# ruiminshen/yolo2-pytorch

Measured on AMD Instinct MI355X. Metric: images/sec (416x416) train+detect, Darknet-19 YOLOv2: value = TRAIN step, batch 64 per GPU (configs[2]) at every N; detect (configs[1]) = roofline.detect_images_per_sec, higher is better.
Workload: dtype f32; 1 GPU; Darknet-19 YOLOv2 20-class train 416x416 batch-64/GPU: fwd + region loss + bwd + SGD (BASELINE configs[2]); classes=20, global_batch=64, parallelism=single GPU, weights=random-init seed 0 (bench_data.randomize)

## Files before the change

include/yolo2_hip.h:

```cpp
#ifndef YOLO2_HIP_H
#define YOLO2_HIP_H

#include <stdint.h>

#ifdef __cplusplus
extern "C" {
#endif

#define Y2_OK 0
#define Y2_EINVAL (-1)
#define Y2_EALIGN (-2)
#define Y2_ENOSUP (-3)

#define Y2_STATS_REPL 32

typedef void* y2_stream_t;

int y2_abi_version(void);
const char* y2_build_info(void);


int y2_pack_weight(const float* w, float* dst, int Cout, int Cin, int ksize, int mode, y2_stream_t stream);

#define Y2_PREP_FPROP 0
// ... 161 lines not shown

int y2_bn_act_fwd(const float* z, const float* scale, const float* shift, float slope, float* y, float* y_pool,
                  int B, int H, int W, int C, int ldz, int ldy, int coff, int ldp, int poff, int out_mode, y2_stream_t stream);

int y2_bn_act_bwd(const float* z, const float* scale, const float* shift, const float* mean, const float* invstd, const float* gamma,
                  float slope, const float* dy_full, int ldf, int foff, int fmode, const float* dy_pool, int ldp, int poff,
                  double* sums, float* dz, int ldd, int B, int H, int W, int C, int ldz, int has_bn, y2_stream_t stream);

int y2_bn_act_fwd_ex(const float* z, const float* scale, const float* shift, float slope, const float* residual, int ldr, float* y, float* y_pool,
                     int B, int H, int W, int C, int ldz, int ldy, int coff, int ldp, int poff, int out_mode, y2_stream_t stream);
int y2_bn_act_bwd_ex(const float* z, const float* scale, const float* shift, const float* mean, const float* invstd, const float* gamma,
                     float slope, const float* dy_full, int ldf, int foff, int fmode, const float* dy_pool, int ldp, int poff,
                     const float* dy_full2, int ld2, const float* residual, int ldr, float* dres, int lddr,
                     double* sums, float* dz, int ldd, int B, int H, int W, int C, int ldz, int has_bn, y2_stream_t stream);

long long y2_wino6_tiles(int32_t B, int32_t H, int32_t W);
int y2_bn_act_bwd_wino6(const float* z, const float* scale, const float* shift, const float* mean, const float* invstd, const float* gamma,
                        float slope, const float* dy_full, int ldf, int foff, double* sums, float* v6, float* m6, float* dz, int ldd,
                        int B, int H, int W, int C, int ldz, int has_bn, y2_stream_t stream);

int y2_maxpool_bwd(const float* x, const float* dy, const float* dy2, float* dx, int B, int H, int W, int C, int ldx, int ldy, int lddx,
                   int ksize, int stride, int pad, int pad_end, y2_stream_t stream);

int y2_colsum(const float* x, long long M, int C, int ld, double* out, y2_stream_t stream);
int y2_f64_to_f32(const double* src, float* dst, int n, double mul, y2_stream_t stream);

int y2_decode_bwd(const float* iou, const float* center_offset, const float* d_iou, const float* d_center_offset, const float* d_size_norm,
                  const float* d_logits, float* d_feature, int boxes, int C, y2_stream_t stream);

int y2_region_loss_fwd(const float* iou, const float* center_offset, const float* size_norm, const float* logits,
// ... 41 lines not shown
```

yolo2-pytorch_amd/_hip.py:

```python
import ctypes
import os
import subprocess

import torch

_HERE = os.path.dirname(os.path.abspath(__file__))
LIB_PATH = os.environ.get('Y2_LIB') or os.path.join(_HERE, 'csrc', 'libyolo2_hip.so')
_lib = None

c_int, c_float, c_void_p = ctypes.c_int, ctypes.c_float, ctypes.c_void_p


class ConvParams(ctypes.Structure):
    _fields_ = [('x', c_void_p), ('w', c_void_p), ('scale', c_void_p), ('shift', c_void_p),
                ('y', c_void_p), ('y_pool', c_void_p), ('stats', c_void_p),
                ('B', ctypes.c_int32), ('H', ctypes.c_int32), ('W', ctypes.c_int32),
                ('Cin', ctypes.c_int32), ('ldx', ctypes.c_int32), ('Cout', ctypes.c_int32), ('ksize', ctypes.c_int32),
                ('ldy', ctypes.c_int32), ('coff', ctypes.c_int32), ('ldp', ctypes.c_int32), ('poff', ctypes.c_int32),
                ('out_mode', ctypes.c_int32), ('slope', c_float), ('tile', ctypes.c_int32),
                ('workspace', c_void_p), ('workspace_bytes', ctypes.c_int64),
                ('residual', c_void_p), ('ldr', ctypes.c_int32), ('stride', ctypes.c_int32), ('pad_plus1', ctypes.c_int32),
                ('transposed', ctypes.c_int32), ('out_h', ctypes.c_int32), ('out_w', ctypes.c_int32), ('algo', ctypes.c_int32),
                ('w_plane', ctypes.c_int64)]

# ... 57 lines not shown
    'y2_filter_visible': [c_void_p, c_void_p, c_int, c_int, c_int, c_int, c_float, c_void_p, c_void_p, c_void_p, c_void_p, c_void_p],
    'y2_iou_matrix': [c_void_p, c_void_p, c_void_p, c_void_p, c_int, c_int, c_int, c_float, c_int, c_void_p, c_void_p],
    'y2_iou_pair': [c_void_p, c_void_p, c_void_p, c_void_p, c_int, c_float, c_void_p, c_void_p],
    'y2_conv_wgrad': [c_void_p, c_void_p, c_void_p, c_int, c_int, c_int, c_int, c_int, c_int, c_int, c_int, c_void_p],
    'y2_conv_wgrad_ex': [c_void_p, c_void_p, c_void_p, c_int, c_int, c_int, c_int, c_int, c_int, c_int, c_int, c_int, c_int, c_void_p],
    'y2_conv0_wgrad_fused': [c_void_p] * 7 + [c_float, c_void_p, c_int, c_void_p, c_void_p] + [c_int] * 7 + [c_void_p],
    'y2_conv0_wgrad': [c_void_p, c_void_p, c_void_p, c_int, c_int, c_int, c_int, c_int, c_int, c_void_p],
    'y2_bn_finalize': [c_void_p, ctypes.c_double, c_void_p, c_void_p, c_void_p, c_void_p, c_float, c_float, c_void_p, c_void_p, c_void_p, c_void_p, c_int, c_void_p, c_void_p],
    'y2_bn_act_fwd': [c_void_p, c_void_p, c_void_p, c_float, c_void_p, c_void_p, c_int, c_int, c_int, c_int, c_int, c_int, c_int, c_int, c_int, c_int, c_void_p],
    'y2_bn_act_bwd': [c_void_p, c_void_p, c_void_p, c_void_p, c_void_p, c_void_p, c_float, c_void_p, c_int, c_int, c_int, c_void_p, c_int, c_int,
                      c_void_p, c_void_p, c_int, c_int, c_int, c_int, c_int, c_int, c_int, c_void_p],
    'y2_bn_act_fwd_ex': [c_void_p, c_void_p, c_void_p, c_float, c_void_p, c_int, c_void_p, c_void_p, c_int, c_int, c_int, c_int, c_int, c_int, c_int, c_int, c_int, c_int, c_void_p],
    'y2_bn_act_bwd_ex': [c_void_p, c_void_p, c_void_p, c_void_p, c_void_p, c_void_p, c_float, c_void_p, c_int, c_int, c_int, c_void_p, c_int, c_int,
                         c_void_p, c_int, c_void_p, c_int, c_void_p, c_int,
                         c_void_p, c_void_p, c_int, c_int, c_int, c_int, c_int, c_int, c_int, c_void_p],
    'y2_wino6_tiles': [c_int, c_int, c_int],
    'y2_bn_act_bwd_wino6': [c_void_p, c_void_p, c_void_p, c_void_p, c_void_p, c_void_p, c_float, c_void_p, c_int, c_int, c_void_p, c_void_p, c_void_p, c_void_p, c_int,
                            c_int, c_int, c_int, c_int, c_int, c_int, c_void_p],
    'y2_maxpool_bwd': [c_void_p, c_void_p, c_void_p, c_void_p, c_int, c_int, c_int, c_int, c_int, c_int, c_int, c_int, c_int, c_int, c_int, c_void_p],
    'y2_colsum': [c_void_p, ctypes.c_longlong, c_int, c_int, c_void_p, c_void_p],
    'y2_dwconv_fwd': [c_void_p, c_void_p, c_void_p, c_void_p, c_float, c_void_p, c_void_p, c_int, c_int, c_int, c_int, c_int, c_int, c_int, c_void_p],
    'y2_dwconv_dgrad': [c_void_p, c_void_p, c_void_p, c_int, c_int, c_int, c_int, c_int, c_int, c_int, c_void_p],
    'y2_dwconv_wgrad': [c_void_p, c_void_p, c_void_p, c_void_p, ctypes.c_longlong, c_int, c_int, c_int, c_int, c_int, c_int, c_int, c_void_p],
    'y2_dwconv_wgrad_workspace_bytes': [c_int, c_int, c_int, c_int, c_int],
    'y2_f64_to_f32': [c_void_p, c_void_p, c_int, ctypes.c_double, c_void_p],
    'y2_decode_bwd': [c_void_p, c_void_p, c_void_p, c_void_p, c_void_p, c_void_p, c_void_p, c_int, c_int, c_void_p],
    'y2_region_loss_fwd': [c_void_p] * 11 + [c_int] * 6 + [c_float] + [c_void_p] * 5 + [c_void_p],
    'y2_region_loss_finalize': [c_void_p, ctypes.c_double, c_int, c_void_p, c_void_p],
    'y2_region_loss_bwd': [c_void_p] * 9 + [c_int] * 6 + [c_float] + [c_void_p] * 5 + [c_void_p] * 4 + [c_void_p],
    'y2_nms_host': [c_void_p, c_void_p, c_void_p, c_void_p, c_void_p, c_int, c_int, c_float, c_int, c_void_p, c_void_p],
# ... 653 lines not shown
```

yolo2-pytorch_amd/csrc/train.hip:

```cpp
#include "common.h"

namespace {

inline int stream_grid(long long total, int block, int cap_mult = 8) {
    long long g = (total + block - 1) / block;
    const long long cap = (long long)Y2_NUM_CU * cap_mult;
    return (int)(g < 1 ? 1 : (g > cap ? cap : g));
}

__global__ void bn_finalize_kernel(const double* __restrict__ stats, double n, const float* gamma, const float* beta,
                                   float* running_mean, float* running_var, float momentum, float eps,
                                   float* scale, float* shift, float* mean_out, float* invstd_out, int C, long long* num_batches_tracked) {
    const int c = blockIdx.x * blockDim.x + threadIdx.x;
    if (c >= C) return;
    if (c == 0 && num_batches_tracked != nullptr) *num_batches_tracked += 1;
    double s1 = 0.0, s2 = 0.0;
    for (int r = 0; r < Y2_STATS_REPL; ++r) { s1 += stats[(size_t)r * 2 * C + c]; s2 += stats[(size_t)r * 2 * C + C + c]; }
    const double mean = s1 / n;
    double var = s2 / n - mean * mean;
    if (var < 0.0) var = 0.0;
    const float invstd = (float)(1.0 / sqrt(var + (double)eps));
    const float s = gamma[c] * invstd;
    scale[c] = s;
    shift[c] = beta[c] - (float)mean * s;
    mean_out[c] = (float)mean;
    invstd_out[c] = invstd;
    if (running_mean != nullptr) {
        const double unbiased = n > 1.0 ? var * n / (n - 1.0) : var;
        running_mean[c] = (1.f - momentum) * running_mean[c] + momentum * (float)mean;
        running_var[c] = (1.f - momentum) * running_var[c] + momentum * (float)unbiased;
    }
}

struct ActArgs {
    const float* z; const float* scale; const float* shift;
    float* y; float* y_pool;
    int B, H, W, C, ldz, ldy, coff, ldp, poff, out_mode;
    float slope;
    const float* res; int ldr;
    y2_fastdiv d_wo, d_ho;
};

__device__ __forceinline__ float act1(float z, float sc, float sh, float slope) {
    const float u = z * sc + sh;
    return u > 0.f ? u : u * slope;
}

__device__ __forceinline__ void act_decode(uint32_t p, const y2_fastdiv& d_wo, const y2_fastdiv& d_ho, int Wo, int Ho, int& b, int& yo, int& xo) {
    const uint32_t r = y2_div(p, d_wo);
    xo = (int)(p - r * (uint32_t)Wo);
    const uint32_t bb = y2_div(r, d_ho);
    yo = (int)(r - bb * (uint32_t)Ho);
    b = (int)bb;
}
// ... 1 lines not shown
template <bool POOL, int CV>
__global__ void bn_act_fwd_kernel(const ActArgs a, long long total) {
    const int Cg = a.C / CV;
    const int Wo = POOL ? a.W / 2 : a.W, Ho = POOL ? a.H / 2 : a.H;
    const long long tid = (long long)blockIdx.x * blockDim.x + threadIdx.x;
    const long long nthreads = (long long)gridDim.x * blockDim.x;
    const int c = (int)(tid % Cg) * CV;
    const uint32_t npix = (uint32_t)(total / Cg), pstep = (uint32_t)(nthreads / Cg);
    float sc[CV], sh[CV];
#pragma unroll
    for (int e = 0; e < CV; ++e) { sc[e] = a.scale ? a.scale[c + e] : 1.f; sh[e] = a.shift ? a.shift[c + e] : 0.f; }
    const bool need_yx = POOL || a.out_mode == 1;
    for (uint32_t p = (uint32_t)(tid / Cg); p < npix; p += pstep) {
        int b = 0, yo = 0, xo = 0;
        if (need_yx) act_decode(p, a.d_wo, a.d_ho, Wo, Ho, b, yo, xo);
        float pm[CV];
#pragma unroll
        for (int q = 0; q < (POOL ? 4 : 1); ++q) {
            const int yy = POOL ? 2 * yo + (q >> 1) : yo, xx = POOL ? 2 * xo + (q & 1) : xo;
            const long long pix = need_yx ? ((long long)b * a.H + yy) * a.W + xx : (long long)p;
            float v[CV];
            if (CV == 4) {
                const f32x4 zz = *reinterpret_cast<const f32x4*>(a.z + pix * a.ldz + c);
                f32x4 rr = {0.f, 0.f, 0.f, 0.f};
                if (a.res != nullptr) rr = *reinterpret_cast<const f32x4*>(a.res + pix * a.ldr + c);
#pragma unroll
                for (int e = 0; e < 4; ++e) { const float u = zz[e] * sc[e] + sh[e] + rr[e]; v[e] = u > 0.f ? u : u * a.slope; }
            } else {
                const float u = a.z[pix * a.ldz + c] * sc[0] + sh[0] + (a.res != nullptr ? a.res[pix * a.ldr + c] : 0.f);
                v[0] = u > 0.f ? u : u * a.slope;
            }
            if (a.y != nullptr) {
                long long o;
                if (a.out_mode == 1) {
                    o = (((long long)b * (a.H >> 1) + (yy >> 1)) * (a.W >> 1) + (xx >> 1)) * a.ldy + a.coff + ((yy & 1) * 2 + (xx & 1)) * a.C + c;
                } else {
                    o = pix * a.ldy + a.coff + c;
                }
                if (CV == 4) { f32x4 w = {v[0], v[1], v[2], v[3]}; *reinterpret_cast<f32x4*>(a.y + o) = w; }
                else a.y[o] = v[0];
            }
#pragma unroll
            for (int e = 0; e < CV; ++e) pm[e] = (q == 0) ? v[e] : fmaxf(pm[e], v[e]);
        }
        if (POOL && a.y_pool != nullptr) {
            const long long o = (long long)p * a.ldp + a.poff + c;
            if (CV == 4) { f32x4 w = {pm[0], pm[1], pm[2], pm[3]}; *reinterpret_cast<f32x4*>(a.y_pool + o) = w; }
            else a.y_pool[o] = pm[0];
        }
    }
}

struct ActBwdArgs {
    const float* z; const float* scale; const float* shift; const float* mean; const float* invstd; const float* gamma;
    const float* dy_full; const float* dy_pool;
    const float* dy_full2; int ld2;
    const float* res; int ldr;
    float* dres; int lddr;
    double* sums;
    float* partial;
    float* block_partial;
    float* dz;
    int B, H, W, C, ldz, ldf, foff, fmode, ldp, poff, ldd;
    float slope;
    double n;
    int has_bn;
    y2_fastdiv d_wo, d_ho;
};

template <bool POOL, int CV, bool APPLY>
// ... 14 lines not shown
        sc[e] = a.scale ? a.scale[c + e] : 1.f; sh[e] = a.shift ? a.shift[c + e] : 0.f;
        mu[e] = a.has_bn ? a.mean[c + e] : 0.f; is[e] = a.has_bn ? a.invstd[c + e] : 1.f;
        if (APPLY && a.has_bn == 1) {
            gs[e] = a.gamma[c + e] * is[e];
            ma[e] = (float)(a.sums[c + e] / a.n);
            mb[e] = (float)(a.sums[a.C + c + e] / a.n);
        } else if (APPLY && a.has_bn == 2) {
            gs[e] = a.gamma[c + e] * is[e]; ma[e] = 0.f; mb[e] = 0.f;
        } else { gs[e] = 1.f; ma[e] = 0.f; mb[e] = 0.f; }
    }
    float s1[CV], s2[CV];
#pragma unroll
    for (int e = 0; e < CV; ++e) { s1[e] = 0.f; s2[e] = 0.f; }

    const uint32_t npix = (uint32_t)(total / Cg), pstep = (uint32_t)(nthreads / Cg);
    const bool need_yx = POOL || a.fmode == 1;
    for (uint32_t p = (uint32_t)(tid / Cg); p < npix; p += pstep) {
        int b = 0, yo = 0, xo = 0;
        if (need_yx) act_decode(p, a.d_wo, a.d_ho, Wo, Ho, b, yo, xo);
        float zv[POOL ? 4 : 1][CV], yv[POOL ? 4 : 1][CV];
        long long pixs[POOL ? 4 : 1];
#pragma unroll
        for (int q = 0; q < (POOL ? 4 : 1); ++q) {
            const int yy = POOL ? 2 * yo + (q >> 1) : yo, xx = POOL ? 2 * xo + (q & 1) : xo;
            pixs[q] = need_yx ? ((long long)b * a.H + yy) * a.W + xx : (long long)p;
            if (CV == 4) {
                const f32x4 zz = *reinterpret_cast<const f32x4*>(a.z + pixs[q] * a.ldz + c);
#pragma unroll
                for (int e = 0; e < 4; ++e) zv[q][e] = zz[e];
            } else zv[q][0] = a.z[pixs[q] * a.ldz + c];
#pragma unroll
            for (int e = 0; e < CV; ++e) yv[q][e] = zv[q][e] * sc[e] + sh[e];
// ... 653 lines not shown
    return (int)(((want + unit - 1) / unit) * unit);
}

}

extern "C" int y2_bn_finalize(const double* stats, double count, const float* gamma, const float* beta,
                              float* running_mean, float* running_var, float momentum, float eps,
                              float* scale, float* shift, float* mean, float* invstd, int C, long long* num_batches_tracked, y2_stream_t stream) {
    if (!stats || !gamma || !beta || !scale || !shift || !mean || !invstd || C <= 0 || count <= 0) return Y2_EINVAL;
    Y2_LAUNCH("bn_finalize_kernel", 0.0, bn_finalize_kernel, dim3(y2_cdiv(C, 256)), dim3(256), 0, y2_s(stream), stats, count, gamma, beta, running_mean, running_var,
                       momentum, eps, scale, shift, mean, invstd, C, num_batches_tracked);
    Y2_LAUNCH_CHECK();
    return Y2_OK;
}

extern "C" int y2_bn_act_fwd_ex(const float* z, const float* scale, const float* shift, float slope, const float* residual, int ldr, float* y, float* y_pool,
                                int B, int H, int W, int C, int ldz, int ldy, int coff, int ldp, int poff, int out_mode, y2_stream_t stream) {
    if (!z || (!y && !y_pool) || B <= 0 || H <= 0 || W <= 0 || C <= 0) return Y2_EINVAL;
    const bool pool = y_pool != nullptr;
    if ((pool || out_mode == 1) && ((H & 1) || (W & 1))) return Y2_EINVAL;
    ActArgs a;
    a.z = z; a.scale = scale; a.shift = shift; a.y = y; a.y_pool = y_pool;
    a.B = B; a.H = H; a.W = W; a.C = C; a.ldz = ldz; a.ldy = ldy; a.coff = coff; a.ldp = ldp; a.poff = poff; a.out_mode = out_mode; a.slope = slope;
    a.res = residual; a.ldr = ldr;
    if (residual != nullptr && ldr < C) return Y2_EINVAL;
    const bool vec = (!residual || (!(ldr & 3) && y2_aligned16(residual))) && !(C & 3) && !(ldz & 3) && (!y || (!(ldy & 3) && !(coff & 3) && y2_aligned16(y))) && (!pool || (!(ldp & 3) && !(poff & 3) && y2_aligned16(y_pool))) && y2_aligned16(z);
    const long long pix = (long long)B * (pool ? H / 2 : H) * (pool ? W / 2 : W);
    if (pix >= 0x7fffffffLL || C > 8192) return Y2_ENOSUP;
    const long long total = pix * (vec ? C / 4 : C);
    const int grid = act_grid(total, vec ? C / 4 : C);
    a.d_wo = y2_make_fastdiv((uint32_t)(pool ? W / 2 : W)); a.d_ho = y2_make_fastdiv((uint32_t)(pool ? H / 2 : H));
    hipStream_t s = y2_s(stream);
    if (pool) { if (vec) Y2_LAUNCH("bn_act_fwd_kernel", 0.0, (bn_act_fwd_kernel<true, 4>), dim3(grid), dim3(256), 0, s, a, total); else Y2_LAUNCH("bn_act_fwd_kernel", 0.0, (bn_act_fwd_kernel<true, 1>), dim3(grid), dim3(256), 0, s, a, total); }
    else { if (vec) Y2_LAUNCH("bn_act_fwd_kernel", 0.0, (bn_act_fwd_kernel<false, 4>), dim3(grid), dim3(256), 0, s, a, total); else Y2_LAUNCH("bn_act_fwd_kernel", 0.0, (bn_act_fwd_kernel<false, 1>), dim3(grid), dim3(256), 0, s, a, total); }
    Y2_LAUNCH_CHECK();
    return Y2_OK;
}

static int bn_act_bwd_impl(const float* z, const float* scale, const float* shift, const float* mean, const float* invstd, const float* gamma,
                           float slope, const float* dy_full, int ldf, int foff, int fmode, const float* dy_pool, int ldp, int poff,
                           const float* dy_full2, int ld2, const float* residual, int ldr, float* dres, int lddr,
                           double* sums, float* dz, int ldd, int B, int H, int W, int C, int ldz, int has_bn, y2_stream_t stream, float* park, long long park_floats) {
    if (!z || (!dy_full && !dy_pool) || !sums || B <= 0 || H <= 0 || W <= 0 || C <= 0) return Y2_EINVAL;
    if (dz == nullptr && dres != nullptr) return Y2_EINVAL;
    if (has_bn < 0 || has_bn > 2 || (has_bn && (!mean || !invstd || !gamma))) return Y2_EINVAL;
    const bool pool = dy_pool != nullptr;
    if ((pool || fmode == 1) && ((H & 1) || (W & 1))) return Y2_EINVAL;
    if (C > 8192) return Y2_ENOSUP;
    ActBwdArgs a;
    a.z = z; a.scale = scale; a.shift = shift; a.mean = mean; a.invstd = invstd; a.gamma = gamma;
    a.dy_full = dy_full; a.dy_pool = dy_pool; a.sums = sums; a.dz = dz;
    a.B = B; a.H = H; a.W = W; a.C = C; a.ldz = ldz; a.ldf = ldf; a.foff = foff; a.fmode = fmode; a.ldp = ldp; a.poff = poff; a.ldd = ldd;
    a.slope = slope; a.n = (double)B * H * W; a.has_bn = has_bn;
    a.dy_full2 = dy_full2; a.ld2 = ld2; a.res = residual; a.ldr = ldr; a.dres = dres; a.lddr = lddr;
    const bool vec = (!dy_full2 || (!(ld2 & 3) && y2_aligned16(dy_full2))) && (!residual || (!(ldr & 3) && y2_aligned16(residual))) && (!dres || (!(lddr & 3) && y2_aligned16(dres))) && !(C & 3) && !(ldz & 3) && (!dz || (!(ldd & 3) && y2_aligned16(dz))) && y2_aligned16(z) &&
                     (!dy_full || (!(ldf & 3) && !(foff & 3) && y2_aligned16(dy_full))) && (!pool || (!(ldp & 3) && !(poff & 3) && y2_aligned16(dy_pool)));
    const int Cg = vec ? C / 4 : C;
    const long long pix = (long long)B * (pool ? H / 2 : H) * (pool ? W / 2 : W);
    if (pix >= 0x7fffffffLL) return Y2_ENOSUP;
    const long long total = pix * Cg;
    const int grid = act_grid(total, Cg);
    a.d_wo = y2_make_fastdiv((uint32_t)(pool ? W / 2 : W)); a.d_ho = y2_make_fastdiv((uint32_t)(pool ? H / 2 : H));
    const size_t lds = (size_t)2 * C * sizeof(float);
    hipStream_t s = y2_s(stream);
    a.partial = nullptr;
    const long long npix = (long long)B * H * W;
    auto overlaps = [&](const float* p, long long floats) {
        if (p == nullptr) return false;
        const char* lo = (const char*)dz; const char* hi = lo + (size_t)npix * ldd * sizeof(float);
        const char* q = (const char*)p;
        return q < hi && lo < q + (size_t)floats * sizeof(float);
    };
    const long long opix = pix;
    const bool aliased = dz != nullptr && (overlaps(z, npix * ldz) || overlaps(dy_full, (fmode == 1 ? npix / 4 : npix) * (long long)ldf) || overlaps(dy_pool, opix * ldp) ||
                                           overlaps(dy_full2, npix * ld2) || overlaps(residual, npix * ldr) || overlaps(dres, npix * lddr));
    a.block_partial = (dz != nullptr && !aliased && !y2_det.on && ldd == C && grid > 16 && (long long)grid * 2 * C <= npix * ldd) ? dz : nullptr;
    if (dz == nullptr && park != nullptr && !y2_det.on && grid > 16 && (long long)grid * 2 * C <= park_floats && y2_aligned16(park)) a.block_partial = park;
    const long long prow = (long long)grid * 256 / Cg;
    if (y2_det.on) {
        if ((size_t)prow * 2 * C * sizeof(float) > y2_det.bytes || prow > 0x7fffffffLL) return Y2_EINVAL;
        a.partial = y2_det.ws;
    }
#define Y2_BWD(POOL, CV)                                                                                             \
    do {                                                                                                             \
        Y2_LAUNCH("bn_act_bwd_kernel", 0.0, (bn_act_bwd_kernel<POOL, CV, false>), dim3(grid), dim3(256), lds, s, a, total);            \
        if (a.partial != nullptr) {                                                                                  \
            const int rc_ = y2_det_reduce_f32(a.partial, (int)prow, (long long)2 * C, (long long)2 * C, sums, nullptr, s);            \
            if (rc_ != Y2_OK) return rc_;                                                                            \
        }                                                                                                            \
// ... 35 lines not shown
    BnWino6Args a;
    a.z = z; a.scale = scale; a.shift = shift; a.mean = mean; a.invstd = invstd; a.gamma = gamma; a.dy = dy_full; a.sums = sums;
    a.v6 = v6; a.m6 = m6; a.dz = dz; a.ldd = ldd;
    a.B = B; a.H = H; a.W = W; a.C = C; a.ldz = ldz; a.ldf = ldf; a.foff = foff; a.has_bn = has_bn; a.slope = slope; a.n = (double)B * H * W;
    a.th = g6.th; a.tw = g6.tw; a.T = (int)g6.T; a.tall = g6.tall; a.wide = g6.wide; a.gx = g6.gx;
    a.d_c = y2_make_fastdiv((uint32_t)C); a.d_tt = y2_make_fastdiv((uint32_t)(g6.th * g6.tw)); a.d_tw = y2_make_fastdiv((uint32_t)g6.tw);
    a.d_tall = y2_make_fastdiv((uint32_t)(g6.tall > 0 ? g6.tall : 1)); a.d_wide = y2_make_fastdiv((uint32_t)(g6.wide > 0 ? g6.wide : 1));
    Y2_LAUNCH("bn_bwd_wino6_kernel", 0.0, bn_bwd_wino6_kernel, dim3((unsigned)y2_cdiv(g6.T * C, 256)), dim3(256), 0, y2_s(stream), a);
    Y2_LAUNCH_CHECK();
    return Y2_OK;
}

extern "C" int y2_bn_act_fwd(const float* z, const float* scale, const float* shift, float slope, float* y, float* y_pool,
                             int B, int H, int W, int C, int ldz, int ldy, int coff, int ldp, int poff, int out_mode, y2_stream_t stream) {
    return y2_bn_act_fwd_ex(z, scale, shift, slope, nullptr, 0, y, y_pool, B, H, W, C, ldz, ldy, coff, ldp, poff, out_mode, stream);
}

extern "C" int y2_bn_act_bwd(const float* z, const float* scale, const float* shift, const float* mean, const float* invstd, const float* gamma,
                             float slope, const float* dy_full, int ldf, int foff, int fmode, const float* dy_pool, int ldp, int poff,
                             double* sums, float* dz, int ldd, int B, int H, int W, int C, int ldz, int has_bn, y2_stream_t stream) {
    return y2_bn_act_bwd_ex(z, scale, shift, mean, invstd, gamma, slope, dy_full, ldf, foff, fmode, dy_pool, ldp, poff, nullptr, 0, nullptr, 0, nullptr, 0,
                            sums, dz, ldd, B, H, W, C, ldz, has_bn, stream);
}

extern "C" int y2_colsum(const float* x, long long M, int C, int ld, double* out, y2_stream_t stream) {
    if (!x || !out || M <= 0 || C <= 0 || ld < C || C > 16384) return Y2_EINVAL;
    int g = 256, r = C;
    while (r) { const int t = g % r; g = r; r = t; }
    const int unit = C / g;
    long long want = (M * C + 256 * 16 - 1) / (256 * 16);
// ... 109 lines not shown
```

yolo2-pytorch_amd/model/train_graph.py:

```python
import ctypes
import os

import numpy as np
import torch
import torch.distributed as dist

import _hip

BWD_STREAMS = int(os.environ.get('Y2_BWD_STREAMS', '2'))
_SIDE = {}


def _side_stream(dev):
    s = _SIDE.get(str(dev))
    if s is None:
        s = torch.cuda.Stream(device=dev)
        _SIDE[str(dev)] = s
    return s


GRAPH_FORK = {'1': True, '0': False}.get(os.environ.get('Y2_GRAPH_FORK', 'auto'), 'auto')
GRAD_F43 = os.environ.get('Y2_GRAD_F43', '1') != '0'
FUSE_WINO6 = os.environ.get('Y2_FUSE_WINO6', '1') != '0'
FUSE_CONV0 = os.environ.get('Y2_FUSE_CONV0', '1') != '0'
DEBUG_TAP = None

SYNC_POSITIVES = True

DP_TAG = '_y2_dp_reduce'


def _sum_over_ranks(t, reducer):
    return bool(reducer(t)) if reducer is not None else False


BN_EPS = 1e-5
BN_MOMENTUM = 0.01
LEAKY = 0.1
_WINO_CHUNK_BYTES = int(os.environ.get('Y2_WINO_CHUNK_MB', '4096')) << 20
# ... 54 lines not shown
    kept = None
    if keep_v and p.algo in (1, 2):
        T = B * ((H + 1) // 2) * ((W + 1) // 2)
        if 16 * T * (cin + cout) * 4 <= _WINO_CHUNK_BYTES and 16 * T * cin * 4 < 0x7fffffff:
            need = L.y2_conv_fwd_workspace_bytes(ctypes.byref(p))
            kept = torch.empty(need // 4 + 4, dtype=torch.float32, device=x.device)
            p.workspace, p.workspace_bytes = kept.data_ptr(), kept.numel() * 4
    if kept is None:
        _hip.conv_workspace(p, dev)
    _hip.check(L.y2_conv_fwd(ctypes.byref(p), st), 'y2_conv_fwd')
    return kept


class _Block(object):
    __slots__ = ('mod', 'name', 'x', 'ldx', 'H', 'W', 'cin', 'cout', 'k', 'z', 'scale', 'shift', 'mean', 'invstd', 'pool',
                 'out_full', 'out_pool', 'out_ld', 'out_off', 'out_mode', 'has_bn', 'slope', 'first', 'wino_v', 'eff')


PRUNE_OPERANDS = os.environ.get('Y2_PRUNE_OPERANDS', '1') != '0'


def _train_operands(dnn, dev, scope=None, only=None, alloc_only=False):
    from model import yolo2 as _yolo2
    if _hip.split_mode() or scope is None:
        only = None
    key = (dev, dnn._weight_versions(), _hip.split_mode(), _hip.WINOGRAD)
    if scope is not None:
        bufs = (dev, scope)
    else:
        cache = getattr(dnn, '_train_cache', None)
        if cache is not None and cache[0] == key:
# ... 171 lines not shown
    arena_used = [0]

    def take(n):
        t = arena[arena_used[0]:arena_used[0] + n]
        arena_used[0] += n
        return t
    blocks = []
    written = []

    def keep_v(h, w, cin, ldx, cout, k):
        if k != 3:
            return False
        with_v, without_v = (_hip.wgrad_choice(B, h, w, cin, ldx, cout, cout, k, hv, dev) for hv in (True, False))
        return not (with_v in (0, 2) or (with_v is None and without_v in (0, 2)))

    def run_block(name, mod, xin, ldx, h, w, pool, out_full=None, out_ld=0, out_off=0, out_mode=0, want_full=True, first=False):
        blk = _Block()
        e = eff[mod]
        L.y2_prof_set_tag(1 + len(blocks))
        cout, cin, k = e.cout, e.cin, mod.kernel_size
        blk.mod, blk.name, blk.x, blk.ldx, blk.H, blk.W, blk.cin, blk.cout, blk.k = mod, name, xin, ldx, h, w, cin, cout, k
        blk.pool, blk.has_bn, blk.slope, blk.first = pool, mod.bn is not None, (LEAKY if mod.has_act else 1.0), first
        blk.wino_v = None
        blk.eff = e
        z = _new(dev, B, h, w, cout)
        stats = take(_hip.STATS_REPL * 2 * cout) if (blk.has_bn and not frozen) else None
        estats = None if det else stats
        if first:
            _hip.check(L.y2_conv0_fwd(_hip.ptr(xin), _hip.ptr(e.w), None, None, _hip.ptr(z), None, _hip.ptr(estats),
                                      B, h, w, cin, cout, cout, 0, 1.0, st), 'y2_conv0_fwd')
        elif mod in prepared:
# ... 21 lines not shown
                bn.running_mean.copy_(e.rm[:e.cout_r])
                bn.running_var.copy_(e.rv[:e.cout_r])
                written.extend(t for t in (bn.num_batches_tracked,) if t is not None)
            else:
                written.extend(t for t in (bn.running_mean, bn.running_var, bn.num_batches_tracked) if t is not None)
        else:
            blk.scale, blk.mean, blk.invstd = None, None, None
            blk.shift = e.bias
        y_full = y_pool = None
        if out_full is not None:
            y_full = out_full
        elif want_full:
            y_full, out_ld, out_off = _new(dev, B, h, w, cout), cout, 0
        if pool:
            y_pool = _new(dev, B, h // 2, w // 2, cout)
        _hip.check(L.y2_bn_act_fwd(_hip.ptr(z), _hip.ptr(blk.scale), _hip.ptr(blk.shift), blk.slope, _hip.ptr(y_full), _hip.ptr(y_pool),
                                   B, h, w, cout, cout, out_ld, out_off, cout, 0, out_mode, st), 'y2_bn_act_fwd')
        blk.out_full, blk.out_pool, blk.out_ld, blk.out_off, blk.out_mode = y_full, y_pool, out_ld, out_off, out_mode
        blocks.append(blk)
        return blk, y_full, y_pool

    cur, ld, h, w = x, cin0, H, W
    full_last = None
    for i, (name, mod, pool) in enumerate(b1):
        last = i == len(b1) - 1
        pool = pool or last
        blk, yf, yp = run_block(name, mod, cur, ld, h, w, pool, want_full=(not pool) or last, first=(i == 0))
        if last:
            full_last, fh, fw = yf, h, w
        if pool:
            cur, h, w = yp, h // 2, w // 2
        else:
            cur = yf
        ld = blk.cout
    c_pt = eff[dnn.passthrough].cout
    c_l2 = eff[b2[-1][1]].cout
    cat = _new(dev, B, h, w, 4 * c_pt + c_l2)
    run_block('passthrough', dnn.passthrough, full_last, full_last.shape[-1], fh, fw, False, out_full=cat, out_ld=cat.shape[-1], out_off=0, out_mode=1)
    for i, (name, mod, pool) in enumerate(b2):
        if i == len(b2) - 1:
            blk, yf, yp = run_block(name, mod, cur, ld, h, w, False, out_full=cat, out_ld=cat.shape[-1], out_off=4 * c_pt)
        else:
# ... 123 lines not shown
        sf, sp = src_full[i], src_pool[i]
        need_dx = bool(getattr(ctx, 'need_dx', False))
        fuse0 = (FUSE_CONV0 and blk.first and i in wg and sf is None and sp is not None and not (h & 1) and not (w & 15)
                 and B * h * w * cout * 4 < 0xffff0000 and not need_dx)
        ready_ops = ctx.prepared.get(blk.mod) if not blk.first else None
        fused6 = None
        if (FUSE_WINO6 and k == 3 and not blk.first and ready_ops is not None and sp is None and sf is not None and sf[3] == 0 and cop == cout and not e.padded
                and i in wg and wg[i][3] == 2 and DEBUG_TAP is None and not _hip.DETERMINISTIC and not _hip.split_mode()):
            hit = _conv(L, st, None, ready_ops['wd'], None, B, h, w, cop, cop, cin, k, cin, u=ready_ops['ud'], grad=True, u_eligible=ready_ops['ud_ok'], u6=ready_ops.get('u6d'), peek=True, dev=dev)
            if hit is not None and hit[0] == 6:
                T6 = int(L.y2_wino6_tiles(B, h, w))
                fused6 = (_new(dev, 36 * T6 * cout), _new(dev, 36 * T6 * cout))
        dz = None if (fuse0 or fused6) else (dzs[i] if i in dzs else _new(dev, B, h, w, cop))
        if DEBUG_TAP is not None:
            DEBUG_TAP(blk.name + ':in', blk.z, blk.shift, sf, sp)
        if fused6:
            _hip.check(L.y2_bn_act_bwd_wino6(_hip.ptr(blk.z), _hip.ptr(blk.scale), _hip.ptr(blk.shift), _hip.ptr(blk.mean), _hip.ptr(blk.invstd),
                                             _hip.ptr(e.gamma) if blk.has_bn else None, blk.slope, _hip.ptr(sf[0]), sf[1], sf[2], _hip.ptr(sums),
                                             _hip.ptr(fused6[0]), _hip.ptr(fused6[1]), None, 0, B, h, w, cout, cout,
                                             (2 if ctx.frozen else 1) if blk.has_bn else 0, st), 'y2_bn_act_bwd_wino6')
        else:
            _hip.check(L.y2_bn_act_bwd(_hip.ptr(blk.z), _hip.ptr(blk.scale), _hip.ptr(blk.shift), _hip.ptr(blk.mean), _hip.ptr(blk.invstd),
                                       _hip.ptr(e.gamma) if blk.has_bn else None, blk.slope,
                                       _hip.ptr(sf[0]) if sf else None, sf[1] if sf else 0, sf[2] if sf else 0, sf[3] if sf else 0,
                                       _hip.ptr(sp), cout, 0, _hip.ptr(sums), _hip.ptr(dz), cop, B, h, w, cout, cout,
                                       (2 if ctx.frozen else 1) if blk.has_bn else 0, st), 'y2_bn_act_bwd')
        if blk.has_bn:
            affine_grads.append((blk.mod.bn.bias, sums_used - 2 * cout, e.cout_r))
            affine_grads.append((blk.mod.bn.weight, sums_used - cout, e.cout_r))
        elif blk.mod.conv.bias is not None:
            affine_grads.append((blk.mod.conv.bias, sums_used - 2 * cout, e.cout_r))
        weight = blk.mod.conv.weight

        def real(dw):
            if not e.padded and cop == cout:
# ... 88 lines not shown
            if blk.name == 'layers3.0':
                dcat = dx
                src_full[i_pass] = (dcat, dcat.shape[-1], 0, 1)
                src_full[idx[dnn._blocks()[1][-1][0]]] = (dcat, dcat.shape[-1], 4 * c_pt, 0)
            elif blk.name == 'passthrough':
                j = n1 - 1
                src_full[j] = (dx, cin, 0, 0)
            elif i == n1 + 1 and blk.name.startswith('layers2.'):
                src_pool[n1 - 1] = dx
            else:
                prod = i - 1
                if blocks[prod].pool:
                    src_pool[prod] = dx
                else:
                    src_full[prod] = (dx, cin, 0, 0)
        blk.z = None
    items, handed = [], []
    gb_all = None
    for prm, off, ln in affine_grads:
        t = buffer_hook(prm) if buffer_hook is not None else None
        if t is None:
            if gb_all is None:
                gb_all = _new(dev, sums_arena.numel())
                items.append((_hip.MULTI_F64_TO_F32, gb_all, sums_arena))
            t = gb_all[off:off + ln]
        else:
            items.append((_hip.MULTI_F64_TO_F32, t, sums_arena[off:off + ln]))
        handed.append((prm, t))
    _hip.multi(items, st)
    for prm, t in handed:
        ready(prm, t)
# ... 1001 lines not shown
```

Measured before the change: 2266 images/sec.

## Record max-pool winning pre-activation in forward to shrink BN backward sums pass

```diff
diff --git a/include/yolo2_hip.h b/include/yolo2_hip.h
--- a/include/yolo2_hip.h
+++ b/include/yolo2_hip.h
@@ -199,6 +199,12 @@
                      const float* dy_full2, int ld2, const float* residual, int ldr, float* dres, int lddr,
                      double* sums, float* dz, int ldd, int B, int H, int W, int C, int ldz, int has_bn, y2_stream_t stream);
 
+int y2_bn_act_fwd_zsel(const float* z, const float* scale, const float* shift, float slope, float* y, float* y_pool, float* z_sel,
+                       int B, int H, int W, int C, int ldz, int ldy, int coff, int ldp, int poff, int out_mode, y2_stream_t stream);
+int y2_bn_act_bwd_zsel(const float* z, const float* z_sel, const float* scale, const float* shift, const float* mean, const float* invstd, const float* gamma,
+                       float slope, const float* dy_pool, int ldp, int poff, double* sums, float* dz, int ldd, int B, int H, int W, int C, int ldz, int has_bn,
+                       y2_stream_t stream);
+
 long long y2_wino6_tiles(int32_t B, int32_t H, int32_t W);
 int y2_bn_act_bwd_wino6(const float* z, const float* scale, const float* shift, const float* mean, const float* invstd, const float* gamma,
                         float slope, const float* dy_full, int ldf, int foff, double* sums, float* v6, float* m6, float* dz, int ldd,
diff --git a/yolo2-pytorch_amd/_hip.py b/yolo2-pytorch_amd/_hip.py
--- a/yolo2-pytorch_amd/_hip.py
+++ b/yolo2-pytorch_amd/_hip.py
@@ -95,6 +95,8 @@
     'y2_bn_act_bwd_ex': [c_void_p, c_void_p, c_void_p, c_void_p, c_void_p, c_void_p, c_float, c_void_p, c_int, c_int, c_int, c_void_p, c_int, c_int,
                          c_void_p, c_int, c_void_p, c_int, c_void_p, c_int,
                          c_void_p, c_void_p, c_int, c_int, c_int, c_int, c_int, c_int, c_int, c_void_p],
+    'y2_bn_act_fwd_zsel': [c_void_p, c_void_p, c_void_p, c_float, c_void_p, c_void_p, c_void_p] + [c_int] * 10 + [c_void_p],
+    'y2_bn_act_bwd_zsel': [c_void_p] * 7 + [c_float, c_void_p, c_int, c_int, c_void_p, c_void_p] + [c_int] * 7 + [c_void_p],
     'y2_wino6_tiles': [c_int, c_int, c_int],
     'y2_bn_act_bwd_wino6': [c_void_p, c_void_p, c_void_p, c_void_p, c_void_p, c_void_p, c_float, c_void_p, c_int, c_int, c_void_p, c_void_p, c_void_p, c_void_p, c_int,
                             c_int, c_int, c_int, c_int, c_int, c_int, c_void_p],
diff --git a/yolo2-pytorch_amd/csrc/train.hip b/yolo2-pytorch_amd/csrc/train.hip
--- a/yolo2-pytorch_amd/csrc/train.hip
+++ b/yolo2-pytorch_amd/csrc/train.hip
@@ -38,6 +38,7 @@
     int B, H, W, C, ldz, ldy, coff, ldp, poff, out_mode;
     float slope;
     const float* res; int ldr;
+    float* z_sel;
     y2_fastdiv d_wo, d_ho;
 };
 
@@ -69,20 +70,21 @@
     for (uint32_t p = (uint32_t)(tid / Cg); p < npix; p += pstep) {
         int b = 0, yo = 0, xo = 0;
         if (need_yx) act_decode(p, a.d_wo, a.d_ho, Wo, Ho, b, yo, xo);
-        float pm[CV];
+        float pm[CV], zs[CV];
 #pragma unroll
         for (int q = 0; q < (POOL ? 4 : 1); ++q) {
             const int yy = POOL ? 2 * yo + (q >> 1) : yo, xx = POOL ? 2 * xo + (q & 1) : xo;
             const long long pix = need_yx ? ((long long)b * a.H + yy) * a.W + xx : (long long)p;
-            float v[CV];
+            float v[CV], zr[CV];
             if (CV == 4) {
                 const f32x4 zz = *reinterpret_cast<const f32x4*>(a.z + pix * a.ldz + c);
                 f32x4 rr = {0.f, 0.f, 0.f, 0.f};
                 if (a.res != nullptr) rr = *reinterpret_cast<const f32x4*>(a.res + pix * a.ldr + c);
 #pragma unroll
-                for (int e = 0; e < 4; ++e) { const float u = zz[e] * sc[e] + sh[e] + rr[e]; v[e] = u > 0.f ? u : u * a.slope; }
+                for (int e = 0; e < 4; ++e) { zr[e] = zz[e]; const float u = zz[e] * sc[e] + sh[e] + rr[e]; v[e] = u > 0.f ? u : u * a.slope; }
             } else {
-                const float u = a.z[pix * a.ldz + c] * sc[0] + sh[0] + (a.res != nullptr ? a.res[pix * a.ldr + c] : 0.f);
+                zr[0] = a.z[pix * a.ldz + c];
+                const float u = zr[0] * sc[0] + sh[0] + (a.res != nullptr ? a.res[pix * a.ldr + c] : 0.f);
                 v[0] = u > 0.f ? u : u * a.slope;
             }
             if (a.y != nullptr) {
@@ -96,19 +98,28 @@
                 else a.y[o] = v[0];
             }
 #pragma unroll
-            for (int e = 0; e < CV; ++e) pm[e] = (q == 0) ? v[e] : fmaxf(pm[e], v[e]);
+            for (int e = 0; e < CV; ++e) {
+                if (q == 0 || v[e] > pm[e]) zs[e] = zr[e];
+                pm[e] = (q == 0) ? v[e] : fmaxf(pm[e], v[e]);
+            }
         }
         if (POOL && a.y_pool != nullptr) {
             const long long o = (long long)p * a.ldp + a.poff + c;
             if (CV == 4) { f32x4 w = {pm[0], pm[1], pm[2], pm[3]}; *reinterpret_cast<f32x4*>(a.y_pool + o) = w; }
             else a.y_pool[o] = pm[0];
         }
+        if (POOL && a.z_sel != nullptr) {
+            const long long o = (long long)p * a.C + c;
+            if (CV == 4) { f32x4 w = {zs[0], zs[1], zs[2], zs[3]}; *reinterpret_cast<f32x4*>(a.z_sel + o) = w; }
+            else a.z_sel[o] = zs[0];
+        }
     }
 }
 
 struct ActBwdArgs {
     const float* z; const float* scale; const float* shift; const float* mean; const float* invstd; const float* gamma;
     const float* dy_full; const float* dy_pool;
+    const float* z_sel;
     const float* dy_full2; int ld2;
     const float* res; int ldr;
     float* dres; int lddr;
@@ -153,8 +164,28 @@
     for (int e = 0; e < CV; ++e) { s1[e] = 0.f; s2[e] = 0.f; }
 
     const uint32_t npix = (uint32_t)(total / Cg), pstep = (uint32_t)(nthreads / Cg);
+    const bool sel = POOL && !APPLY && a.z_sel != nullptr;
+    if (sel) {
+        for (uint32_t p = (uint32_t)(tid / Cg); p < npix; p += pstep) {
+            float zs[CV], dp[CV];
+            const long long o = (long long)p * a.ldp + a.poff + c;
+            if (CV == 4) {
+                const f32x4 zz = *reinterpret_cast<const f32x4*>(a.z_sel + (long long)p * a.C + c);
+                const f32x4 d = *reinterpret_cast<const f32x4*>(a.dy_pool + o);
+#pragma unroll
+                for (int e = 0; e < 4; ++e) { zs[e] = zz[e]; dp[e] = d[e]; }
+            } else { zs[0] = a.z_sel[(long long)p * a.C + c]; dp[0] = a.dy_pool[o]; }
+#pragma unroll
+            for (int e = 0; e < CV; ++e) {
+                const float u = zs[e] * sc[e] + sh[e];
+                const float ge = dp[e] * (u > 0.f ? 1.f : a.slope);
+                const float zh = (zs[e] - mu[e]) * is[e];
+                s1[e] += ge; s2[e] += ge * zh;
+            }
+        }
+    }
     const bool need_yx = POOL || a.fmode == 1;
-    for (uint32_t p = (uint32_t)(tid / Cg); p < npix; p += pstep) {
+    for (uint32_t p = (uint32_t)(tid / Cg); !sel && p < npix; p += pstep) {
         int b = 0, yo = 0, xo = 0;
         if (need_yx) act_decode(p, a.d_wo, a.d_ho, Wo, Ho, b, yo, xo);
         float zv[POOL ? 4 : 1][CV], yv[POOL ? 4 : 1][CV];
@@ -838,17 +869,18 @@
     return Y2_OK;
 }
 
-extern "C" int y2_bn_act_fwd_ex(const float* z, const float* scale, const float* shift, float slope, const float* residual, int ldr, float* y, float* y_pool,
-                                int B, int H, int W, int C, int ldz, int ldy, int coff, int ldp, int poff, int out_mode, y2_stream_t stream) {
+static int bn_act_fwd_impl(const float* z, const float* scale, const float* shift, float slope, const float* residual, int ldr, float* y, float* y_pool, float* z_sel,
+                           int B, int H, int W, int C, int ldz, int ldy, int coff, int ldp, int poff, int out_mode, y2_stream_t stream) {
     if (!z || (!y && !y_pool) || B <= 0 || H <= 0 || W <= 0 || C <= 0) return Y2_EINVAL;
     const bool pool = y_pool != nullptr;
+    if (z_sel != nullptr && !pool) return Y2_EINVAL;
     if ((pool || out_mode == 1) && ((H & 1) || (W & 1))) return Y2_EINVAL;
     ActArgs a;
     a.z = z; a.scale = scale; a.shift = shift; a.y = y; a.y_pool = y_pool;
     a.B = B; a.H = H; a.W = W; a.C = C; a.ldz = ldz; a.ldy = ldy; a.coff = coff; a.ldp = ldp; a.poff = poff; a.out_mode = out_mode; a.slope = slope;
-    a.res = residual; a.ldr = ldr;
+    a.res = residual; a.ldr = ldr; a.z_sel = z_sel;
     if (residual != nullptr && ldr < C) return Y2_EINVAL;
-    const bool vec = (!residual || (!(ldr & 3) && y2_aligned16(residual))) && !(C & 3) && !(ldz & 3) && (!y || (!(ldy & 3) && !(coff & 3) && y2_aligned16(y))) && (!pool || (!(ldp & 3) && !(poff & 3) && y2_aligned16(y_pool))) && y2_aligned16(z);
+    const bool vec = (!residual || (!(ldr & 3) && y2_aligned16(residual))) && (!z_sel || y2_aligned16(z_sel)) && !(C & 3) && !(ldz & 3) && (!y || (!(ldy & 3) && !(coff & 3) && y2_aligned16(y))) && (!pool || (!(ldp & 3) && !(poff & 3) && y2_aligned16(y_pool))) && y2_aligned16(z);
     const long long pix = (long long)B * (pool ? H / 2 : H) * (pool ? W / 2 : W);
     if (pix >= 0x7fffffffLL || C > 8192) return Y2_ENOSUP;
     const long long total = pix * (vec ? C / 4 : C);
@@ -861,23 +893,36 @@
     return Y2_OK;
 }
 
+extern "C" int y2_bn_act_fwd_ex(const float* z, const float* scale, const float* shift, float slope, const float* residual, int ldr, float* y, float* y_pool,
+                                int B, int H, int W, int C, int ldz, int ldy, int coff, int ldp, int poff, int out_mode, y2_stream_t stream) {
+    return bn_act_fwd_impl(z, scale, shift, slope, residual, ldr, y, y_pool, nullptr, B, H, W, C, ldz, ldy, coff, ldp, poff, out_mode, stream);
+}
+
+extern "C" int y2_bn_act_fwd_zsel(const float* z, const float* scale, const float* shift, float slope, float* y, float* y_pool, float* z_sel,
+                                  int B, int H, int W, int C, int ldz, int ldy, int coff, int ldp, int poff, int out_mode, y2_stream_t stream) {
+    if (z_sel == nullptr) return Y2_EINVAL;
+    return bn_act_fwd_impl(z, scale, shift, slope, nullptr, 0, y, y_pool, z_sel, B, H, W, C, ldz, ldy, coff, ldp, poff, out_mode, stream);
+}
+
 static int bn_act_bwd_impl(const float* z, const float* scale, const float* shift, const float* mean, const float* invstd, const float* gamma,
                            float slope, const float* dy_full, int ldf, int foff, int fmode, const float* dy_pool, int ldp, int poff,
                            const float* dy_full2, int ld2, const float* residual, int ldr, float* dres, int lddr,
-                           double* sums, float* dz, int ldd, int B, int H, int W, int C, int ldz, int has_bn, y2_stream_t stream, float* park, long long park_floats) {
+                           double* sums, float* dz, int ldd, int B, int H, int W, int C, int ldz, int has_bn, y2_stream_t stream, float* park, long long park_floats,
+                           const float* z_sel = nullptr) {
     if (!z || (!dy_full && !dy_pool) || !sums || B <= 0 || H <= 0 || W <= 0 || C <= 0) return Y2_EINVAL;
     if (dz == nullptr && dres != nullptr) return Y2_EINVAL;
+    if (z_sel != nullptr && (!dy_pool || dy_full || dy_full2 || residual)) return Y2_EINVAL;
     if (has_bn < 0 || has_bn > 2 || (has_bn && (!mean || !invstd || !gamma))) return Y2_EINVAL;
     const bool pool = dy_pool != nullptr;
     if ((pool || fmode == 1) && ((H & 1) || (W & 1))) return Y2_EINVAL;
     if (C > 8192) return Y2_ENOSUP;
     ActBwdArgs a;
     a.z = z; a.scale = scale; a.shift = shift; a.mean = mean; a.invstd = invstd; a.gamma = gamma;
-    a.dy_full = dy_full; a.dy_pool = dy_pool; a.sums = sums; a.dz = dz;
+    a.dy_full = dy_full; a.dy_pool = dy_pool; a.z_sel = z_sel; a.sums = sums; a.dz = dz;
     a.B = B; a.H = H; a.W = W; a.C = C; a.ldz = ldz; a.ldf = ldf; a.foff = foff; a.fmode = fmode; a.ldp = ldp; a.poff = poff; a.ldd = ldd;
     a.slope = slope; a.n = (double)B * H * W; a.has_bn = has_bn;
     a.dy_full2 = dy_full2; a.ld2 = ld2; a.res = residual; a.ldr = ldr; a.dres = dres; a.lddr = lddr;
-    const bool vec = (!dy_full2 || (!(ld2 & 3) && y2_aligned16(dy_full2))) && (!residual || (!(ldr & 3) && y2_aligned16(residual))) && (!dres || (!(lddr & 3) && y2_aligned16(dres))) && !(C & 3) && !(ldz & 3) && (!dz || (!(ldd & 3) && y2_aligned16(dz))) && y2_aligned16(z) &&
+    const bool vec = (!dy_full2 || (!(ld2 & 3) && y2_aligned16(dy_full2))) && (!residual || (!(ldr & 3) && y2_aligned16(residual))) && (!dres || (!(lddr & 3) && y2_aligned16(dres))) && (!z_sel || y2_aligned16(z_sel)) && !(C & 3) && !(ldz & 3) && (!dz || (!(ldd & 3) && y2_aligned16(dz))) && y2_aligned16(z) &&
                      (!dy_full || (!(ldf & 3) && !(foff & 3) && y2_aligned16(dy_full))) && (!pool || (!(ldp & 3) && !(poff & 3) && y2_aligned16(dy_pool)));
     const int Cg = vec ? C / 4 : C;
     const long long pix = (long long)B * (pool ? H / 2 : H) * (pool ? W / 2 : W);
@@ -896,7 +941,7 @@
         return q < hi && lo < q + (size_t)floats * sizeof(float);
     };
     const long long opix = pix;
-    const bool aliased = dz != nullptr && (overlaps(z, npix * ldz) || overlaps(dy_full, (fmode == 1 ? npix / 4 : npix) * (long long)ldf) || overlaps(dy_pool, opix * ldp) ||
+    const bool aliased = dz != nullptr && (overlaps(z, npix * ldz) || overlaps(z_sel, opix * C) || overlaps(dy_full, (fmode == 1 ? npix / 4 : npix) * (long long)ldf) || overlaps(dy_pool, opix * ldp) ||
                                            overlaps(dy_full2, npix * ld2) || overlaps(residual, npix * ldr) || overlaps(dres, npix * lddr));
     a.block_partial = (dz != nullptr && !aliased && !y2_det.on && ldd == C && grid > 16 && (long long)grid * 2 * C <= npix * ldd) ? dz : nullptr;
     if (dz == nullptr && park != nullptr && !y2_det.on && grid > 16 && (long long)grid * 2 * C <= park_floats && y2_aligned16(park)) a.block_partial = park;
@@ -962,6 +1007,14 @@
 extern "C" int y2_bn_act_fwd(const float* z, const float* scale, const float* shift, float slope, float* y, float* y_pool,
                              int B, int H, int W, int C, int ldz, int ldy, int coff, int ldp, int poff, int out_mode, y2_stream_t stream) {
     return y2_bn_act_fwd_ex(z, scale, shift, slope, nullptr, 0, y, y_pool, B, H, W, C, ldz, ldy, coff, ldp, poff, out_mode, stream);
+}
+
+extern "C" int y2_bn_act_bwd_zsel(const float* z, const float* z_sel, const float* scale, const float* shift, const float* mean, const float* invstd, const float* gamma,
+                                  float slope, const float* dy_pool, int ldp, int poff, double* sums, float* dz, int ldd, int B, int H, int W, int C, int ldz, int has_bn,
+                                  y2_stream_t stream) {
+    if (z_sel == nullptr || dy_pool == nullptr) return Y2_EINVAL;
+    return bn_act_bwd_impl(z, scale, shift, mean, invstd, gamma, slope, nullptr, 0, 0, 0, dy_pool, ldp, poff, nullptr, 0, nullptr, 0, nullptr, 0,
+                           sums, dz, ldd, B, H, W, C, ldz, has_bn, stream, nullptr, 0, z_sel);
 }
 
 extern "C" int y2_bn_act_bwd(const float* z, const float* scale, const float* shift, const float* mean, const float* invstd, const float* gamma,
diff --git a/yolo2-pytorch_amd/model/train_graph.py b/yolo2-pytorch_amd/model/train_graph.py
--- a/yolo2-pytorch_amd/model/train_graph.py
+++ b/yolo2-pytorch_amd/model/train_graph.py
@@ -23,6 +23,7 @@
 GRAD_F43 = os.environ.get('Y2_GRAD_F43', '1') != '0'
 FUSE_WINO6 = os.environ.get('Y2_FUSE_WINO6', '1') != '0'
 FUSE_CONV0 = os.environ.get('Y2_FUSE_CONV0', '1') != '0'
+FOLD_BN_SUMS = os.environ.get('Y2_FOLD_BN_SUMS', '1') != '0'
 DEBUG_TAP = None
 
 SYNC_POSITIVES = True
@@ -107,7 +108,7 @@
 
 class _Block(object):
     __slots__ = ('mod', 'name', 'x', 'ldx', 'H', 'W', 'cin', 'cout', 'k', 'z', 'scale', 'shift', 'mean', 'invstd', 'pool',
-                 'out_full', 'out_pool', 'out_ld', 'out_off', 'out_mode', 'has_bn', 'slope', 'first', 'wino_v', 'eff')
+                 'out_full', 'out_pool', 'out_ld', 'out_off', 'out_mode', 'has_bn', 'slope', 'first', 'wino_v', 'eff', 'z_sel')
 
 
 PRUNE_OPERANDS = os.environ.get('Y2_PRUNE_OPERANDS', '1') != '0'
@@ -309,7 +310,7 @@
         with_v, without_v = (_hip.wgrad_choice(B, h, w, cin, ldx, cout, cout, k, hv, dev) for hv in (True, False))
         return not (with_v in (0, 2) or (with_v is None and without_v in (0, 2)))
 
-    def run_block(name, mod, xin, ldx, h, w, pool, out_full=None, out_ld=0, out_off=0, out_mode=0, want_full=True, first=False):
+    def run_block(name, mod, xin, ldx, h, w, pool, out_full=None, out_ld=0, out_off=0, out_mode=0, want_full=True, first=False, pool_only=False):
         blk = _Block()
         e = eff[mod]
         L.y2_prof_set_tag(1 + len(blocks))
@@ -361,8 +362,14 @@
             y_full, out_ld, out_off = _new(dev, B, h, w, cout), cout, 0
         if pool:
             y_pool = _new(dev, B, h // 2, w // 2, cout)
-        _hip.check(L.y2_bn_act_fwd(_hip.ptr(z), _hip.ptr(blk.scale), _hip.ptr(blk.shift), blk.slope, _hip.ptr(y_full), _hip.ptr(y_pool),
-                                   B, h, w, cout, cout, out_ld, out_off, cout, 0, out_mode, st), 'y2_bn_act_fwd')
+        blk.z_sel = None
+        if pool and pool_only and FOLD_BN_SUMS and DEBUG_TAP is None:
+            blk.z_sel = _new(dev, B, h // 2, w // 2, cout)
+            _hip.check(L.y2_bn_act_fwd_zsel(_hip.ptr(z), _hip.ptr(blk.scale), _hip.ptr(blk.shift), blk.slope, _hip.ptr(y_full), _hip.ptr(y_pool), _hip.ptr(blk.z_sel),
+                                            B, h, w, cout, cout, out_ld, out_off, cout, 0, out_mode, st), 'y2_bn_act_fwd_zsel')
+        else:
+            _hip.check(L.y2_bn_act_fwd(_hip.ptr(z), _hip.ptr(blk.scale), _hip.ptr(blk.shift), blk.slope, _hip.ptr(y_full), _hip.ptr(y_pool),
+                                       B, h, w, cout, cout, out_ld, out_off, cout, 0, out_mode, st), 'y2_bn_act_fwd')
         blk.out_full, blk.out_pool, blk.out_ld, blk.out_off, blk.out_mode = y_full, y_pool, out_ld, out_off, out_mode
         blocks.append(blk)
         return blk, y_full, y_pool
@@ -372,7 +379,7 @@
     for i, (name, mod, pool) in enumerate(b1):
         last = i == len(b1) - 1
         pool = pool or last
-        blk, yf, yp = run_block(name, mod, cur, ld, h, w, pool, want_full=(not pool) or last, first=(i == 0))
+        blk, yf, yp = run_block(name, mod, cur, ld, h, w, pool, want_full=(not pool) or last, first=(i == 0), pool_only=not last)
         if last:
             full_last, fh, fw = yf, h, w
         if pool:
@@ -526,11 +533,16 @@
         dz = None if (fuse0 or fused6) else (dzs[i] if i in dzs else _new(dev, B, h, w, cop))
         if DEBUG_TAP is not None:
             DEBUG_TAP(blk.name + ':in', blk.z, blk.shift, sf, sp)
+        zsel = blk.z_sel if (sf is None and sp is not None) else None
         if fused6:
             _hip.check(L.y2_bn_act_bwd_wino6(_hip.ptr(blk.z), _hip.ptr(blk.scale), _hip.ptr(blk.shift), _hip.ptr(blk.mean), _hip.ptr(blk.invstd),
                                              _hip.ptr(e.gamma) if blk.has_bn else None, blk.slope, _hip.ptr(sf[0]), sf[1], sf[2], _hip.ptr(sums),
                                              _hip.ptr(fused6[0]), _hip.ptr(fused6[1]), None, 0, B, h, w, cout, cout,
                                              (2 if ctx.frozen else 1) if blk.has_bn else 0, st), 'y2_bn_act_bwd_wino6')
+        elif zsel is not None:
+            _hip.check(L.y2_bn_act_bwd_zsel(_hip.ptr(blk.z), _hip.ptr(zsel), _hip.ptr(blk.scale), _hip.ptr(blk.shift), _hip.ptr(blk.mean), _hip.ptr(blk.invstd),
+                                            _hip.ptr(e.gamma) if blk.has_bn else None, blk.slope, _hip.ptr(sp), cout, 0, _hip.ptr(sums), _hip.ptr(dz), cop,
+                                            B, h, w, cout, cout, (2 if ctx.frozen else 1) if blk.has_bn else 0, st), 'y2_bn_act_bwd_zsel')
         else:
             _hip.check(L.y2_bn_act_bwd(_hip.ptr(blk.z), _hip.ptr(blk.scale), _hip.ptr(blk.shift), _hip.ptr(blk.mean), _hip.ptr(blk.invstd),
                                        _hip.ptr(e.gamma) if blk.has_bn else None, blk.slope,
@@ -649,7 +661,7 @@
                     src_pool[prod] = dx
                 else:
                     src_full[prod] = (dx, cin, 0, 0)
-        blk.z = None
+        blk.z = blk.z_sel = None
     items, handed = [], []
     gb_all = None
     for prm, off, ln in affine_grads:
```

Result: no change. 2278 images/sec, median of 6 (+0.5%).
